# thierrydumas/autoencoder_based_image_compression

Measured on AMD Instinct MI355X. Metric: Mpixels/s encode+decode (Kodak 768x512 luma), bitstream bit-exact, higher is better.
Workload: dtype f32; 1 GPU; kodak_512x768_luma_batch24_per_gpu_bin_width_1.0_lossless_roundtrip; height=512, width=768, truncated_unary_length=10, idx_map_exception=67, parallelism=single GPU, coder=device, 64 maps per wavefront, encode + decode + compare

## Files before the change

autoencoder_based_image_compression_amd/csrc/hip/latent.hip:

```cpp
#include "latent_body.h"

#include <cstdlib>

namespace {
constexpr int WAVES = 2;
constexpr int TM = WAVES * 32;
constexpr int SYM_STRIDE = TM + 2;

template <bool GDN_IN, bool IGDN_OUT>
__global__ __launch_bounds__(WAVES * 64) void latent_kernel(const float* x, const float* __restrict__ gamma_in,
                                                     const float* __restrict__ beta_in, const float* __restrict__ map_mean,
                                                     const float* __restrict__ bin_widths, const float* __restrict__ gamma_out,
                                                     const float* __restrict__ beta_out, float* y_out,
                                                     float* shifted_out, float* t_out,
                                                     int16_t* __restrict__ symbols, unsigned int* __restrict__ nonzero,
                                                     unsigned int* __restrict__ checks, long rows, int hw) {
    __shared__ __attribute__((aligned(16))) float Xs[TM * EAE_XS_STRIDE];
    __shared__ int16_t Sy[EAE_C * SYM_STRIDE];
    const int tid = threadIdx.x, lane = tid & 63, wm = tid >> 6;
    const long row0 = (long)blockIdx.x * TM;
    for (int i = tid; i < TM * (EAE_C / 4); i += WAVES * 64) {
        const int r = i >> 5, q = i & 31;
        float4 v = make_float4(0.f, 0.f, 0.f, 0.f);
        if (row0 + r < rows) v = *reinterpret_cast<const float4*>(x + (size_t)(row0 + r) * EAE_C + 4 * q);
        float* dst = Xs + r * EAE_XS_STRIDE + 4 * q;
        dst[0] = v.x; dst[1] = v.y; dst[2] = v.z; dst[3] = v.w;
    }
    __syncthreads();
    const int col0 = lane & 31;
    const long img0 = row0 / hw;
    const int pix0 = (int)(row0 - img0 * hw);
    const bool simple = hw >= TM;
    f32x16 d[4];
    if (GDN_IN) {
        gdn_denominator<4>(Xs, wm, lane, gamma_in, 0, d);
        __syncthreads();
    }
    unsigned int bad = 0, not_quantized = 0, altered = 0;
#pragma unroll
    for (int t = 0; t < 4; ++t) {
        const int c = col0 + 32 * t;
        const float m = map_mean ? map_mean[c] : 0.f;
        const float bw = bin_widths[c];
        const float bt = GDN_IN ? beta_in[c] : 0.f;
#pragma unroll
        for (int r = 0; r < 16; ++r) {
            const int mrow = wm * 32 + acc_row32(r, lane);
            const long row = row0 + mrow;
            float yv = Xs[mrow * EAE_XS_STRIDE + c];
            if (GDN_IN) yv = gdn_apply(yv, d[t][r], bt, false);
            const float centered = yv - m;
            const float rr = round_half_even(centered / bw);
            const float cq = bw * rr;
            const float rs = round_half_even(cq / bw);
            const float shifted = cq + m;
            if (row < rows) {
                if (!(fabsf(rs) < 32768.f)) bad++;
                if (!(fabs((double)cq - (double)centered) < 1.5e-10)) not_quantized++;
                if (!((float)(int16_t)(int)rs * bw == centered)) altered++;
                if (y_out) y_out[(size_t)row * EAE_C + c] = yv;
                if (shifted_out) shifted_out[(size_t)row * EAE_C + c] = shifted;
                if (cq != 0.f && nonzero) {
                    const long img = simple ? img0 + (pix0 + mrow >= hw ? 1 : 0) : row / hw;
                    nonzero[img * EAE_C + c] = 1u;
                }
            }
            Xs[mrow * EAE_XS_STRIDE + c] = shifted;
            Sy[c * SYM_STRIDE + mrow] = (int16_t)(int)rs;
        }
    }
    if (checks) {
        if (bad) atomicAdd(&checks[0], bad);
        if (not_quantized) atomicAdd(&checks[1], not_quantized);
        if (altered) atomicAdd(&checks[2], altered);
    }
    __syncthreads();
    if (symbols) {
        for (int i = tid; i < EAE_C * TM; i += WAVES * 64) {
            const int ch = i / TM, px = i % TM;
            const long row = row0 + px;
            if (row < rows) {
                const bool next = pix0 + px >= hw;
                const long img = simple ? img0 + (next ? 1 : 0) : row / hw;
                const int pix = simple ? pix0 + px - (next ? hw : 0) : (int)(row % hw);
                symbols[((size_t)img * EAE_C + ch) * hw + pix] = Sy[ch * SYM_STRIDE + px];
            }
        }
    }
    if (IGDN_OUT) {
        gdn_denominator<4>(Xs, wm, lane, gamma_out, 0, d);
#pragma unroll
        for (int t = 0; t < 4; ++t) {
            const int c = col0 + 32 * t;
            const float bt = beta_out[c];
#pragma unroll
            for (int r = 0; r < 16; ++r) {
                const int mrow = wm * 32 + acc_row32(r, lane);
                if (row0 + mrow < rows)
                    t_out[(size_t)(row0 + mrow) * EAE_C + c] = gdn_apply(Xs[mrow * EAE_XS_STRIDE + c], d[t][r], bt, true);
            }
        }
    }
}

template <bool GDN_IN, bool IGDN_OUT>
__global__ __launch_bounds__(64) void latent_wave_kernel(const float* x, const float* __restrict__ gamma_in,
                                                         const float* __restrict__ beta_in, const float* __restrict__ map_mean,
                                                         const float* __restrict__ bin_widths, const float* __restrict__ gamma_out,
                                                         const float* __restrict__ beta_out, float* y_out,
                                                         float* shifted_out, float* t_out,
                                                         int16_t* __restrict__ symbols, unsigned int* __restrict__ nonzero,
                                                         unsigned int* __restrict__ checks, long rows, int hw) {
    __shared__ __attribute__((aligned(16))) float vec[4 * EAE_C];
    const int lane = threadIdx.x, hi = lane >> 5, lj = lane & 31;
    {
        const float2 z = make_float2(0.f, 0.f);
        *reinterpret_cast<float2*>(vec + 2 * lane) = GDN_IN ? *reinterpret_cast<const float2*>(beta_in + 2 * lane) : z;
        *reinterpret_cast<float2*>(vec + EAE_C + 2 * lane) = IGDN_OUT ? *reinterpret_cast<const float2*>(beta_out + 2 * lane) : z;
        *reinterpret_cast<float2*>(vec + 2 * EAE_C + 2 * lane) = map_mean ? *reinterpret_cast<const float2*>(map_mean + 2 * lane) : z;
        *reinterpret_cast<float2*>(vec + 3 * EAE_C + 2 * lane) = *reinterpret_cast<const float2*>(bin_widths + 2 * lane);
    }
    const long row = (long)blockIdx.x * 32 + lj;
    const bool valid = row < rows;
    const long img = row / hw;
    const int pix = (int)(row - img * hw);
    const float* xrow = x + (size_t)(valid ? row : 0) * EAE_C + 4 * hi;
    f32x16 v[4];
#pragma unroll
    for (int t = 0; t < 4; ++t)
#pragma unroll
        for (int g = 0; g < 4; ++g) {
            const float4 q = valid ? *reinterpret_cast<const float4*>(xrow + 32 * t + 8 * g) : make_float4(0.f, 0.f, 0.f, 0.f);
            v[t][4 * g + 0] = q.x; v[t][4 * g + 1] = q.y; v[t][4 * g + 2] = q.z; v[t][4 * g + 3] = q.w;
        }
    __syncthreads();
    const LatentOut o{y_out, shifted_out, t_out, symbols, nonzero, checks};
    wave_latent_body<GDN_IN, IGDN_OUT>(v, vec, gamma_in, gamma_out, o, valid, img, pix, hw, lane);
}

template <bool GDN_IN, bool IGDN_OUT>
__global__ __launch_bounds__(256) void latent_quarter_kernel(const float* x, const float* __restrict__ gamma_in,
                                                             const float* __restrict__ beta_in, const float* __restrict__ map_mean,
                                                             const float* __restrict__ bin_widths, const float* __restrict__ gamma_out,
                                                             const float* __restrict__ beta_out, float* y_out,
                                                             float* shifted_out, float* t_out,
                                                             int16_t* __restrict__ symbols, unsigned int* __restrict__ nonzero,
                                                             unsigned int* __restrict__ checks, long rows, int hw) {
    __shared__ __attribute__((aligned(16))) float vec[4 * EAE_C];
    __shared__ __attribute__((aligned(16))) float xch[4 * 4 * 64 * 4];
    __shared__ unsigned int tally[4][3];
    const int tid = threadIdx.x, lane = tid & 63, hi = lane >> 5, lj = lane & 31;
    const int w = __builtin_amdgcn_readfirstlane(tid >> 6);
    if (tid < EAE_C) {
        vec[tid] = GDN_IN ? beta_in[tid] : 0.f;
        vec[EAE_C + tid] = IGDN_OUT ? beta_out[tid] : 0.f;
        vec[2 * EAE_C + tid] = map_mean ? map_mean[tid] : 0.f;
        vec[3 * EAE_C + tid] = bin_widths[tid];
    }
    const long row = (long)blockIdx.x * 32 + lj;
    const bool valid = row < rows;
    const long img = row / hw;
    const int pix = (int)(row - img * hw);
    const int cw = 32 * w + 4 * hi;
    const size_t obase = (size_t)(valid ? row : 0) * EAE_C + cw;
    f32x16 own;
#pragma unroll
    for (int g = 0; g < 4; ++g) {
        const float4 q = valid ? *reinterpret_cast<const float4*>(x + obase + 8 * g) : make_float4(0.f, 0.f, 0.f, 0.f);
        own[4 * g + 0] = q.x; own[4 * g + 1] = q.y; own[4 * g + 2] = q.z; own[4 * g + 3] = q.w;
    }
    float4* slot = reinterpret_cast<float4*>(xch) + lane;
    f32x16 full[4];
#define EAE_Q_EXCHANGE()                                                                                                 \
    {                                                                                                                    \
        const f32x16 sq = squares_for_mfma(own);                                                                         \
        _Pragma("unroll") for (int g = 0; g < 4; ++g)                                                                    \
            slot[(4 * w + g) * 64] = make_float4(sq[4 * g], sq[4 * g + 1], sq[4 * g + 2], sq[4 * g + 3]);                \
        __syncthreads();                                                                                                 \
        _Pragma("unroll") for (int t = 0; t < 4; ++t)                                                                    \
            _Pragma("unroll") for (int g = 0; g < 4; ++g) {                                                              \
                const float4 q = slot[(4 * t + g) * 64];                                                                 \
                full[t][4 * g + 0] = q.x; full[t][4 * g + 1] = q.y; full[t][4 * g + 2] = q.z; full[t][4 * g + 3] = q.w;  \
            }                                                                                                            \
    }
    if (GDN_IN) {
        EAE_Q_EXCHANGE()
        f32x16 d[1] = {quarter_denominator<8>(full, gamma_in, w, lane)};
#pragma unroll
        for (int g = 0; g < 4; ++g) {
            const float4 bt = *reinterpret_cast<const float4*>(vec + cw + 8 * g);
            d[0][4 * g + 0] = d[0][4 * g + 0] + bt.x;
            d[0][4 * g + 1] = d[0][4 * g + 1] + bt.y;
            d[0][4 * g + 2] = d[0][4 * g + 2] + bt.z;
            d[0][4 * g + 3] = d[0][4 * g + 3] + bt.w;
        }
        const f32x16 xn[1] = {own};
        gdn_tile<1, false, false>(xn, d, [&](int, int g, float4 y) {
            own[4 * g + 0] = y.x; own[4 * g + 1] = y.y; own[4 * g + 2] = y.z; own[4 * g + 3] = y.w;
        });
    } else {
        __syncthreads();
    }
    const long img0 = ((long)blockIdx.x * 32) / hw;
    const bool one_image = __all(!valid || img == img0) != 0;
    const __amdgpu_buffer_rsrc_t sym_rsrc = __builtin_amdgcn_make_buffer_rsrc(
        symbols ? symbols + (size_t)img0 * EAE_C * hw : nullptr, 0, symbols ? 0x7FFFFFFF : 0, 0x00020000);
    const int sym_lane = valid ? (int)((((img - img0) * EAE_C + 4 * hi) * hw + pix) * 2) : -1;
    unsigned int bad = 0, not_quantized = 0, altered = 0, flag_bits = 0;
#pragma unroll
    for (int g = 0; g < 4; ++g) {
        const float4 m4 = *reinterpret_cast<const float4*>(vec + 2 * EAE_C + cw + 8 * g);
        const float4 b4 = *reinterpret_cast<const float4*>(vec + 3 * EAE_C + cw + 8 * g);
        const float mm[4] = {m4.x, m4.y, m4.z, m4.w}, bw[4] = {b4.x, b4.y, b4.z, b4.w};
        float sh[4];
#pragma unroll
        for (int q = 0; q < 4; ++q) {
            const float yv = own[4 * g + q];
            const float centered = yv - mm[q];
            const float rr = round_half_even(centered / bw[q]);
            const float cq = bw[q] * rr;
            const float rs = round_half_even(cq / bw[q]);
            sh[q] = cq + mm[q];
            if (valid) {
                if (!(fabsf(rs) < 32768.f)) bad++;
                if (!(fabs((double)cq - (double)centered) < 1.5e-10)) not_quantized++;
                if (!((float)(int16_t)(int)rs * bw[q] == centered)) altered++;
            }
            const bool nz = valid && cq != 0.f;
            if (nonzero) {
                if (one_image) {
                    const unsigned long long any = __ballot(nz);
                    if ((unsigned int)any) flag_bits |= 1u << (8 * g + q);
                    if ((unsigned int)(any >> 32)) flag_bits |= 1u << (8 * g + 4 + q);
                } else if (nz) {
                    nonzero[img * EAE_C + cw + 8 * g + q] = 1u;
                }
            }
            if (symbols)
                __builtin_amdgcn_raw_buffer_store_b16((short)(int16_t)(int)rs, sym_rsrc, sym_lane, (32 * w + 8 * g + q) * hw * 2, 0);
        }
        if (valid && y_out)
            *reinterpret_cast<float4*>(y_out + obase + 8 * g) = make_float4(own[4 * g], own[4 * g + 1], own[4 * g + 2], own[4 * g + 3]);
        if (valid && shifted_out) *reinterpret_cast<float4*>(shifted_out + obase + 8 * g) = make_float4(sh[0], sh[1], sh[2], sh[3]);
        own[4 * g + 0] = sh[0]; own[4 * g + 1] = sh[1]; own[4 * g + 2] = sh[2]; own[4 * g + 3] = sh[3];
    }
    if (nonzero && one_image && lane < 32 && ((flag_bits >> lane) & 1u)) nonzero[img0 * EAE_C + 32 * w + lane] = 1u;
#ifndef EAE_LATENT_NOCHECKS
    if (checks) {
#pragma unroll
        for (int off = 32; off > 0; off >>= 1) {
            bad += __shfl_down(bad, off, 64);
            not_quantized += __shfl_down(not_quantized, off, 64);
            altered += __shfl_down(altered, off, 64);
        }
        if (lane == 0) { tally[w][0] = bad; tally[w][1] = not_quantized; tally[w][2] = altered; }
    }
#endif
    if (IGDN_OUT) {
        if (GDN_IN) __syncthreads();
        EAE_Q_EXCHANGE()
        f32x16 d[1] = {quarter_denominator<8>(full, gamma_out, w, lane)};
#pragma unroll
        for (int g = 0; g < 4; ++g) {
            const float4 bt = *reinterpret_cast<const float4*>(vec + EAE_C + cw + 8 * g);
            d[0][4 * g + 0] = d[0][4 * g + 0] + bt.x;
            d[0][4 * g + 1] = d[0][4 * g + 1] + bt.y;
            d[0][4 * g + 2] = d[0][4 * g + 2] + bt.z;
            d[0][4 * g + 3] = d[0][4 * g + 3] + bt.w;
        }
        const f32x16 xn[1] = {own};
        gdn_tile<1, true, false>(xn, d, [&](int, int g, float4 y) {
            if (valid) *reinterpret_cast<float4*>(t_out + obase + 8 * g) = y;
        });
    }
#ifndef EAE_LATENT_NOCHECKS
    if (checks) {
        if (!IGDN_OUT) __syncthreads();
        if (tid < 3) {
            const unsigned int sum = tally[0][tid] + tally[1][tid] + tally[2][tid] + tally[3][tid];
            if (sum) atomicAdd(&checks[tid], sum);
        }
    }
#endif
#undef EAE_Q_EXCHANGE
}
}

extern "C" int eae_hip_latent_stage(const float* x, const float* gamma_in_packed, const float* beta_in, const float* map_mean,
                                    const float* bin_widths, const float* gamma_out_packed, const float* beta_out, float* y_out,
                                    float* shifted_out, float* t_out, int16_t* symbols_planar, uint32_t* nonzero_flags,
                                    uint32_t* checks, int n, int hw, void* stream) {
    if (!x || !bin_widths || n <= 0 || hw <= 0) return EAE_HIP_BAD_ARGUMENT;
    if ((gamma_in_packed == nullptr) != (beta_in == nullptr)) return EAE_HIP_BAD_ARGUMENT;
    if ((gamma_out_packed == nullptr) != (beta_out == nullptr) || (gamma_out_packed && !t_out)) return EAE_HIP_BAD_ARGUMENT;
    const long rows = (long)n * hw;
    hipStream_t s = (hipStream_t)stream;
    char form = g_eae_launch_options.latent;
    if (form == 'q' && hw > (1 << 21)) form = 'w';
    if (form != 'l') {
        const unsigned wgrid = (unsigned)((rows + 31) / 32);
#define EAE_LATENT_W(A_, B_)                                                                                              \
        {                                                                                                                \
            if (form == 'q')                                                                                             \
                hipLaunchKernelGGL((latent_quarter_kernel<A_, B_>), dim3(wgrid), dim3(256), 0, s, x, gamma_in_packed, beta_in, map_mean,  \
                                   bin_widths, gamma_out_packed, beta_out, y_out, shifted_out, t_out, symbols_planar, nonzero_flags, checks, rows, hw); \
            else                                                                                                         \
                hipLaunchKernelGGL((latent_wave_kernel<A_, B_>), dim3(wgrid), dim3(64), 0, s, x, gamma_in_packed, beta_in, map_mean,  \
                                   bin_widths, gamma_out_packed, beta_out, y_out, shifted_out, t_out, symbols_planar, nonzero_flags, checks, rows, hw); \
        }
        if (gamma_in_packed && gamma_out_packed) EAE_LATENT_W(true, true)
        else if (gamma_in_packed) EAE_LATENT_W(true, false)
        else if (gamma_out_packed) EAE_LATENT_W(false, true)
        else EAE_LATENT_W(false, false)
#undef EAE_LATENT_W
        EAE_HIP_CHECK_LAUNCH();
        return EAE_HIP_OK;
    }
    const unsigned grid = (unsigned)((rows + TM - 1) / TM);
#define EAE_LATENT(A_, B_)                                                                                               \
    hipLaunchKernelGGL((latent_kernel<A_, B_>), dim3(grid), dim3(WAVES * 64), 0, s, x, gamma_in_packed, beta_in, map_mean, bin_widths, \
                       gamma_out_packed, beta_out, y_out, shifted_out, t_out, symbols_planar, nonzero_flags, checks, rows, hw)
    if (gamma_in_packed && gamma_out_packed) EAE_LATENT(true, true);
    else if (gamma_in_packed) EAE_LATENT(true, false);
    else if (gamma_out_packed) EAE_LATENT(false, true);
    else EAE_LATENT(false, false);
#undef EAE_LATENT
    EAE_HIP_CHECK_LAUNCH();
    return EAE_HIP_OK;
}
```

autoencoder_based_image_compression_amd/csrc/hip/latent_body.h:

```cpp
#pragma once
#include "common.h"

#ifndef EAE_LATENT_RING
#define EAE_LATENT_RING 8
#endif
#ifdef EAE_LATENT_TRACE
#define LAT_MARK(i_) { const long long t_ = clock64(); if (o.checks && lane == 0) atomicAdd(&o.checks[16 + (i_)], (unsigned int)((t_ - lat_last) >> 4)); lat_last = t_; }
#else
#define LAT_MARK(i_)
#endif

template <bool INVERSE>
__device__ __forceinline__ void wave_gdn_inplace(f32x16 (&x)[4], const float* beta_lds, const float* __restrict__ gamma_packed,
                                                 int lane) {
    constexpr int RING = EAE_LATENT_RING;
    const int hi = lane >> 5, lj = lane & 31;
    const __amdgpu_buffer_rsrc_t g_rsrc = __builtin_amdgcn_make_buffer_rsrc(
        const_cast<float*>(gamma_packed), 0, (int)(EAE_C * EAE_C * sizeof(float)), 0x00020000);
    const int g_lane = (hi * EAE_C + lj * 4) * 4;
    f32x16 d[4];
#pragma unroll
    for (int t = 0; t < 4; ++t)
#pragma unroll
        for (int r = 0; r < 16; ++r) d[t][r] = 0.f;
    float4 ring[RING];
#define EAE_L_LOAD(dst_, kk_)                                                                                            \
    {                                                                                                                    \
        const u32x4 v_ = __builtin_amdgcn_raw_buffer_load_b128(g_rsrc, g_lane + (kk_) * 2 * EAE_C * 4, 0, 0);            \
        dst_ = make_float4(__uint_as_float(v_.x), __uint_as_float(v_.y), __uint_as_float(v_.z), __uint_as_float(v_.w));  \
    }
#pragma unroll
    for (int i = 0; i < RING; ++i) EAE_L_LOAD(ring[i], i)
#pragma unroll
    for (int t = 0; t < 4; ++t) {
#pragma unroll
        for (int g = 0; g < 4; ++g) {
            float s0 = x[t][4 * g + 0], s1 = x[t][4 * g + 1], s2 = x[t][4 * g + 2], s3 = x[t][4 * g + 3];
            swap_halves(s0, s1);
            swap_halves(s2, s3);
            const float xs[4] = {s0, s2, s1, s3};
#pragma unroll
            for (int e = 0; e < 4; ++e) {
                const int kk = 16 * t + 4 * g + e;
                const float x2 = xs[e] * xs[e];
                const float4 gq = ring[kk % RING];
                d[0] = mfma32(gq.x, x2, d[0]);
                d[1] = mfma32(gq.y, x2, d[1]);
                d[2] = mfma32(gq.z, x2, d[2]);
                d[3] = mfma32(gq.w, x2, d[3]);
                if (kk + RING < EAE_C / 2) { EAE_L_LOAD(ring[kk % RING], kk + RING) }
            }
        }
    }
#undef EAE_L_LOAD
#pragma unroll
    for (int t = 0; t < 4; ++t)
#pragma unroll
        for (int g = 0; g < 4; ++g) {
            const float4 bt = *reinterpret_cast<const float4*>(beta_lds + 32 * t + 8 * g + 4 * hi);
            d[t][4 * g + 0] = d[t][4 * g + 0] + bt.x;
            d[t][4 * g + 1] = d[t][4 * g + 1] + bt.y;
            d[t][4 * g + 2] = d[t][4 * g + 2] + bt.z;
            d[t][4 * g + 3] = d[t][4 * g + 3] + bt.w;
        }
    gdn_tile<4, INVERSE>(x, d, [&](int t, int g, float4 y) {
        x[t][4 * g + 0] = y.x; x[t][4 * g + 1] = y.y; x[t][4 * g + 2] = y.z; x[t][4 * g + 3] = y.w;
    });
}


struct LatentOut {
    float* y_out;
    float* shifted_out;
    float* t_out;
    int16_t* symbols;
    unsigned int* nonzero;
    unsigned int* checks;
};

template <bool GDN_IN, bool IGDN_OUT>
__device__ __forceinline__ void wave_latent_body(f32x16 (&v)[4], const float* vec, const float* __restrict__ gamma_in,
                                                 const float* __restrict__ gamma_out, const LatentOut& o, bool valid, long img,
                                                 int pix, int hw, int lane) {
    const int hi = lane >> 5;
#ifdef EAE_LATENT_TRACE
    long long lat_last = clock64();
#endif
    if (GDN_IN) wave_gdn_inplace<false>(v, vec, gamma_in, lane);
    LAT_MARK(0)
    unsigned int bad = 0, not_quantized = 0, altered = 0;
    const size_t obase = ((size_t)(valid ? img : 0) * hw + (valid ? pix : 0)) * EAE_C + 4 * hi;
#pragma unroll
    for (int t = 0; t < 4; ++t)
#pragma unroll
        for (int g = 0; g < 4; ++g) {
            const int c0 = 32 * t + 8 * g + 4 * hi;
            const float4 m4 = *reinterpret_cast<const float4*>(vec + 2 * EAE_C + c0);
            const float4 b4 = *reinterpret_cast<const float4*>(vec + 3 * EAE_C + c0);
            const float mm[4] = {m4.x, m4.y, m4.z, m4.w}, bw[4] = {b4.x, b4.y, b4.z, b4.w};
            float sh[4];
#pragma unroll
            for (int q = 0; q < 4; ++q) {
                const float yv = v[t][4 * g + q];
                const float centered = yv - mm[q];
                const float rr = round_half_even(centered / bw[q]);
                const float cq = bw[q] * rr;
                const float rs = round_half_even(cq / bw[q]);
                sh[q] = cq + mm[q];
                if (valid) {
                    if (!(fabsf(rs) < 32768.f)) bad++;
                    if (!(fabs((double)cq - (double)centered) < 1.5e-10)) not_quantized++;
                    if (!((float)(int16_t)(int)rs * bw[q] == centered)) altered++;
                    if (cq != 0.f && o.nonzero) o.nonzero[img * EAE_C + c0 + q] = 1u;
                    if (o.symbols) o.symbols[((size_t)img * EAE_C + c0 + q) * hw + pix] = (int16_t)(int)rs;
                }
            }
            if (valid && o.y_out)
                *reinterpret_cast<float4*>(o.y_out + obase + 32 * t + 8 * g) =
                    make_float4(v[t][4 * g], v[t][4 * g + 1], v[t][4 * g + 2], v[t][4 * g + 3]);
            if (valid && o.shifted_out) *reinterpret_cast<float4*>(o.shifted_out + obase + 32 * t + 8 * g) = make_float4(sh[0], sh[1], sh[2], sh[3]);
            v[t][4 * g + 0] = sh[0]; v[t][4 * g + 1] = sh[1]; v[t][4 * g + 2] = sh[2]; v[t][4 * g + 3] = sh[3];
        }
    LAT_MARK(1)
    if (o.checks) {
        if (bad) atomicAdd(&o.checks[0], bad);
        if (not_quantized) atomicAdd(&o.checks[1], not_quantized);
        if (altered) atomicAdd(&o.checks[2], altered);
    }
    if (IGDN_OUT) {
        wave_gdn_inplace<true>(v, vec + EAE_C, gamma_out, lane);
        LAT_MARK(2)
        if (valid) {
#pragma unroll
            for (int t = 0; t < 4; ++t)
#pragma unroll
                for (int g = 0; g < 4; ++g)
                    *reinterpret_cast<float4*>(o.t_out + obase + 32 * t + 8 * g) =
                        make_float4(v[t][4 * g], v[t][4 * g + 1], v[t][4 * g + 2], v[t][4 * g + 3]);
        }
        LAT_MARK(3)
    }
}


template <int RING>
__device__ __forceinline__ f32x16 quarter_denominator(const f32x16 (&x2)[4], const float* __restrict__ gamma_packed, int w, int lane) {
    const int hi = lane >> 5, lj = lane & 31;
    const __amdgpu_buffer_rsrc_t g_rsrc = __builtin_amdgcn_make_buffer_rsrc(
        const_cast<float*>(gamma_packed), 0, (int)(EAE_C * EAE_C * sizeof(float)), 0x00020000);
    const int g_lane = (hi * EAE_C + lj * 4 + w) * 4;
    f32x16 d;
#pragma unroll
    for (int r = 0; r < 16; ++r) d[r] = 0.f;
    float ring[RING];
#pragma unroll
    for (int i = 0; i < RING; ++i) ring[i] = __uint_as_float(__builtin_amdgcn_raw_buffer_load_b32(g_rsrc, g_lane, i * 2 * EAE_C * 4, 0));
#pragma unroll
    for (int kk = 0; kk < EAE_C / 2; ++kk) {
        d = mfma32(ring[kk % RING], x2[kk >> 4][kk & 15], d);
        if (kk + RING < EAE_C / 2)
            ring[kk % RING] = __uint_as_float(__builtin_amdgcn_raw_buffer_load_b32(g_rsrc, g_lane, (kk + RING) * 2 * EAE_C * 4, 0));
    }
    return d;
}

__device__ __forceinline__ f32x16 squares_for_mfma(const f32x16& v) {
    f32x16 r;
#pragma unroll
    for (int g = 0; g < 4; ++g) {
        float s0 = v[4 * g + 0], s1 = v[4 * g + 1], s2 = v[4 * g + 2], s3 = v[4 * g + 3];
        swap_halves(s0, s1);
        swap_halves(s2, s3);
        r[4 * g + 0] = s0 * s0; r[4 * g + 1] = s2 * s2; r[4 * g + 2] = s1 * s1; r[4 * g + 3] = s3 * s3;
    }
    return r;
}
```

Baseline: 3026 Mpixels/s.

## Tier quantiser checks by wave-uniform range tests and count them via ballots

```diff
diff --git a/autoencoder_based_image_compression_amd/csrc/hip/latent.hip b/autoencoder_based_image_compression_amd/csrc/hip/latent.hip
--- a/autoencoder_based_image_compression_amd/csrc/hip/latent.hip
+++ b/autoencoder_based_image_compression_amd/csrc/hip/latent.hip
@@ -139,7 +139,7 @@
 }
 
 template <bool GDN_IN, bool IGDN_OUT>
-__global__ __launch_bounds__(256) void latent_quarter_kernel(const float* x, const float* __restrict__ gamma_in,
+__global__ __launch_bounds__(256, 5) void latent_quarter_kernel(const float* x, const float* __restrict__ gamma_in,
                                                              const float* __restrict__ beta_in, const float* __restrict__ map_mean,
                                                              const float* __restrict__ bin_widths, const float* __restrict__ gamma_out,
                                                              const float* __restrict__ beta_out, float* y_out,
@@ -195,7 +195,7 @@
             d[0][4 * g + 3] = d[0][4 * g + 3] + bt.w;
         }
         const f32x16 xn[1] = {own};
-        gdn_tile<1, false, false>(xn, d, [&](int, int g, float4 y) {
+        gdn_tile<1, false, true>(xn, d, [&](int, int g, float4 y) {
             own[4 * g + 0] = y.x; own[4 * g + 1] = y.y; own[4 * g + 2] = y.z; own[4 * g + 3] = y.w;
         });
     } else {
@@ -207,54 +207,70 @@
         symbols ? symbols + (size_t)img0 * EAE_C * hw : nullptr, 0, symbols ? 0x7FFFFFFF : 0, 0x00020000);
     const int sym_lane = valid ? (int)((((img - img0) * EAE_C + 4 * hi) * hw + pix) * 2) : -1;
     unsigned int bad = 0, not_quantized = 0, altered = 0, flag_bits = 0;
+    f32x16 rr;
+    float rr_max = 0.f;
 #pragma unroll
     for (int g = 0; g < 4; ++g) {
         const float4 m4 = *reinterpret_cast<const float4*>(vec + 2 * EAE_C + cw + 8 * g);
         const float4 b4 = *reinterpret_cast<const float4*>(vec + 3 * EAE_C + cw + 8 * g);
         const float mm[4] = {m4.x, m4.y, m4.z, m4.w}, bw[4] = {b4.x, b4.y, b4.z, b4.w};
-        float sh[4];
-#pragma unroll
-        for (int q = 0; q < 4; ++q) {
-            const float yv = own[4 * g + q];
-            const float centered = yv - mm[q];
-            const float rr = round_half_even(centered / bw[q]);
-            const float cq = bw[q] * rr;
-            const float rs = round_half_even(cq / bw[q]);
-            sh[q] = cq + mm[q];
-            if (valid) {
-                if (!(fabsf(rs) < 32768.f)) bad++;
-                if (!(fabs((double)cq - (double)centered) < 1.5e-10)) not_quantized++;
-                if (!((float)(int16_t)(int)rs * bw[q] == centered)) altered++;
-            }
-            const bool nz = valid && cq != 0.f;
-            if (nonzero) {
-                if (one_image) {
-                    const unsigned long long any = __ballot(nz);
-                    if ((unsigned int)any) flag_bits |= 1u << (8 * g + q);
-                    if ((unsigned int)(any >> 32)) flag_bits |= 1u << (8 * g + 4 + q);
-                } else if (nz) {
-                    nonzero[img * EAE_C + cw + 8 * g + q] = 1u;
-                }
-            }
-            if (symbols)
-                __builtin_amdgcn_raw_buffer_store_b16((short)(int16_t)(int)rs, sym_rsrc, sym_lane, (32 * w + 8 * g + q) * hw * 2, 0);
-        }
         if (valid && y_out)
             *reinterpret_cast<float4*>(y_out + obase + 8 * g) = make_float4(own[4 * g], own[4 * g + 1], own[4 * g + 2], own[4 * g + 3]);
-        if (valid && shifted_out) *reinterpret_cast<float4*>(shifted_out + obase + 8 * g) = make_float4(sh[0], sh[1], sh[2], sh[3]);
-        own[4 * g + 0] = sh[0]; own[4 * g + 1] = sh[1]; own[4 * g + 2] = sh[2]; own[4 * g + 3] = sh[3];
+#pragma unroll
+        for (int q = 0; q < 4; ++q) {
+            const float centered = own[4 * g + q] - mm[q];
+            rr[4 * g + q] = round_half_even(centered / bw[q]);
+            rr_max = quantiser_rr_max(rr_max, rr[4 * g + q]);
+            own[4 * g + q] = centered;
+        }
+        __builtin_amdgcn_sched_barrier(0);
+    }
+    const int tier = quantiser_tier(bin_widths_in_range(vec + 3 * EAE_C, lane), rr_max);
+    auto rest = [&](auto tier_) {
+        constexpr int TIER = decltype(tier_)::value;
+#pragma unroll
+        for (int g = 0; g < 4; ++g) {
+            const float4 m4 = *reinterpret_cast<const float4*>(vec + 2 * EAE_C + cw + 8 * g);
+            const float4 b4 = *reinterpret_cast<const float4*>(vec + 3 * EAE_C + cw + 8 * g);
+            const float mm[4] = {m4.x, m4.y, m4.z, m4.w}, bw[4] = {b4.x, b4.y, b4.z, b4.w};
+            float sh[4];
+#pragma unroll
+            for (int q = 0; q < 4; ++q) {
+                float cq, rs;
+                quantiser_checks<TIER>(own[4 * g + q], rr[4 * g + q], bw[q], cq, rs, bad, not_quantized, altered);
+                sh[q] = cq + mm[q];
+                const unsigned long long any = __builtin_amdgcn_ballot_w64(cq != 0.f);
+                flag_bits |= any_bit((unsigned int)any) << (8 * g + q) | any_bit((unsigned int)(any >> 32)) << (8 * g + 4 + q);
+                __builtin_amdgcn_raw_buffer_store_b16((short)(int16_t)(int)rs, sym_rsrc, sym_lane, (32 * w + 8 * g + q) * hw * 2, 0);
+            }
+            if (shifted_out) *reinterpret_cast<float4*>(shifted_out + obase + 8 * g) = make_float4(sh[0], sh[1], sh[2], sh[3]);
+            own[4 * g + 0] = sh[0]; own[4 * g + 1] = sh[1]; own[4 * g + 2] = sh[2]; own[4 * g + 3] = sh[3];
+            asm volatile("" : "+s"(bad), "+s"(not_quantized), "+s"(altered), "+s"(flag_bits));
+            __builtin_amdgcn_sched_barrier(0);
+        }
+    };
+    if (valid) {
+        if (tier == 2) rest(std::integral_constant<int, 2>{});
+        else if (tier == 1) rest(std::integral_constant<int, 1>{});
+        else rest(std::integral_constant<int, 0>{});
+    }
+    bad = __builtin_amdgcn_readfirstlane(bad);
+    not_quantized = __builtin_amdgcn_readfirstlane(not_quantized);
+    altered = __builtin_amdgcn_readfirstlane(altered);
+    flag_bits = __builtin_amdgcn_readfirstlane(flag_bits);
+    if (nonzero && !one_image && valid) {
+#pragma unroll
+        for (int g = 0; g < 4; ++g) {
+            const float4 b4 = *reinterpret_cast<const float4*>(vec + 3 * EAE_C + cw + 8 * g);
+            const float bw[4] = {b4.x, b4.y, b4.z, b4.w};
+#pragma unroll
+            for (int q = 0; q < 4; ++q)
+                if (bw[q] * rr[4 * g + q] != 0.f) nonzero[img * EAE_C + cw + 8 * g + q] = 1u;
+        }
     }
     if (nonzero && one_image && lane < 32 && ((flag_bits >> lane) & 1u)) nonzero[img0 * EAE_C + 32 * w + lane] = 1u;
 #ifndef EAE_LATENT_NOCHECKS
-    if (checks) {
-#pragma unroll
-        for (int off = 32; off > 0; off >>= 1) {
-            bad += __shfl_down(bad, off, 64);
-            not_quantized += __shfl_down(not_quantized, off, 64);
-            altered += __shfl_down(altered, off, 64);
-        }
-        if (lane == 0) { tally[w][0] = bad; tally[w][1] = not_quantized; tally[w][2] = altered; }
-    }
+    if (checks && lane == 0) { tally[w][0] = bad; tally[w][1] = not_quantized; tally[w][2] = altered; }
 #endif
     if (IGDN_OUT) {
         if (GDN_IN) __syncthreads();
@@ -269,7 +285,7 @@
             d[0][4 * g + 3] = d[0][4 * g + 3] + bt.w;
         }
         const f32x16 xn[1] = {own};
-        gdn_tile<1, true, false>(xn, d, [&](int, int g, float4 y) {
+        gdn_tile<1, true, true>(xn, d, [&](int, int g, float4 y) {
             if (valid) *reinterpret_cast<float4*>(t_out + obase + 8 * g) = y;
         });
     }
diff --git a/autoencoder_based_image_compression_amd/csrc/hip/latent_body.h b/autoencoder_based_image_compression_amd/csrc/hip/latent_body.h
--- a/autoencoder_based_image_compression_amd/csrc/hip/latent_body.h
+++ b/autoencoder_based_image_compression_amd/csrc/hip/latent_body.h
@@ -1,5 +1,7 @@
 #pragma once
 #include "common.h"
+
+#include <type_traits>
 
 #ifndef EAE_LATENT_RING
 #define EAE_LATENT_RING 8
@@ -68,6 +70,39 @@
     });
 }
 
+
+#define EAE_Q_BW_MIN 0x1p-100f
+#define EAE_Q_BW_END 0x1p107f
+#define EAE_Q_RR_END 0x1p21f
+#define EAE_Q_NOT_QUANTIZED 0x1.49da80p-33f
+static_assert((double)EAE_Q_NOT_QUANTIZED >= 1.5e-10 && (double)0x1.49da7ep-33f < 1.5e-10, "the float neighbours of 1.5e-10");
+
+__device__ __forceinline__ bool bin_widths_in_range(const float* bw_lds, int lane) {
+    const float2 b = *reinterpret_cast<const float2*>(bw_lds + 2 * lane);
+    const bool in = b.x >= EAE_Q_BW_MIN && b.x < EAE_Q_BW_END && b.y >= EAE_Q_BW_MIN && b.y < EAE_Q_BW_END;
+    return __builtin_amdgcn_ballot_w64(!in) == 0ull;
+}
+
+__device__ __forceinline__ float quantiser_rr_max(float m, float rr) { return __builtin_elementwise_maximum(m, __builtin_fabsf(rr)); }
+__device__ __forceinline__ int quantiser_tier(bool widths_in_range, float rr_max) {
+    if (!widths_in_range) return 0;
+    if (__builtin_amdgcn_ballot_w64(!(rr_max < 32768.f)) == 0ull) return 2;
+    return __builtin_amdgcn_ballot_w64(!(rr_max < EAE_Q_RR_END)) == 0ull ? 1 : 0;
+}
+
+__device__ __forceinline__ unsigned int any_bit(unsigned int word) { return ((unsigned int)__builtin_popcount(word) + 31u) >> 5; }
+
+template <int TIER>
+__device__ __forceinline__ void quantiser_checks(float centered, float rr, float bw, float& cq, float& rs,
+                                                 unsigned int& bad, unsigned int& not_quantized, unsigned int& altered) {
+    cq = bw * rr;
+    rs = TIER == 0 ? round_half_even(cq / bw) : rr;
+    if (TIER < 2) bad += __builtin_popcountll(__builtin_amdgcn_ballot_w64(!(__builtin_fabsf(rs) < 32768.f)));
+    not_quantized += __builtin_popcountll(TIER == 0 ? __builtin_amdgcn_ballot_w64(!(fabs((double)cq - (double)centered) < 1.5e-10))
+                                                    : __builtin_amdgcn_ballot_w64(!(__builtin_fabsf(cq - centered) < EAE_Q_NOT_QUANTIZED)));
+    altered += __builtin_popcountll(TIER < 2 ? __builtin_amdgcn_ballot_w64(!((float)(int16_t)(int)rs * bw == centered))
+                                             : __builtin_amdgcn_ballot_w64(!(cq == centered)));
+}
 
 struct LatentOut {
     float* y_out;
```

New measurement: 3028 Mpixels/s (median of 2 runs). About the same (+0.1%).
